# cinemere/evacuation

Measured on NVIDIA B200. Metric: pedestrian-steps/s, higher is better.
Workload: dtype f32

## Files before the change

evacuation_b200/_native.py:

```python
from __future__ import annotations

import ctypes as C
import os

from . import build as _build
from .build import LIB_PATH

EVAC_ABI_VERSION = 5
NUM_EPISODE_STATS = 9
EPISODE_STAT_KEYS = (
    "episode_intrinsic_reward", "episode_status_reward", "episode_reward", "episode_length",
    "escaped_pedestrians", "exiting_pedestrians", "following_pedestrians", "viscek_pedestrians",
    "overall_timesteps",
)

POS = {"abs": 0, "rel": 1, "grav": 2}
STAT = {"no": 0, "ohe": 1, "cat": 2}
OBS = {"Dict": 0, "Box": 1}
PREC = {"fp32": 0, "fp64": 1}
AGENT = {"table": 0, "random": 1, "rotating": 2, "wacuum": 3}
SEARCH = {"auto": 0, "brute": 1, "cells": 2}


class EvacConfig(C.Structure):
# ... 27 lines not shown
    _fields_ = [
        ("num_envs", C.c_int32), ("obs", C.c_void_p),
        ("norm_mean", C.c_void_p), ("norm_var", C.c_void_p), ("norm_count", C.c_void_p), ("obs_norm", C.c_void_p),
        ("norm_eps", C.c_float), ("norm_clip", C.c_float),
        ("embedding", C.c_void_p), ("mean", C.c_void_p), ("value", C.c_void_p), ("action", C.c_void_p),
        ("action_clipped", C.c_void_p), ("logprob", C.c_void_p), ("entropy", C.c_void_p), ("given_action", C.c_void_p),
        ("sample", C.c_int32), ("training", C.c_int32), ("seed", C.c_uint64), ("offset", C.c_uint64),
        ("offset_device", C.c_void_p), ("env_index_offset", C.c_int64),
    ]


_P = C.c_void_p
SIGNATURES = {
    "evac_abi_version": (C.c_int32, []),
    "evac_last_error": (C.c_char_p, []),
    "evac_build_id": (C.c_char_p, []),
    "evac_default_config": (C.c_int, [C.POINTER(EvacConfig)]),
    "evac_create": (C.c_int, [C.POINTER(EvacConfig), C.c_int32, C.c_int32, C.c_uint64, C.c_int64, C.POINTER(_P)]),
    "evac_destroy": (C.c_int, [_P]),
    "evac_obs_dim": (C.c_int32, [_P]),
    "evac_num_envs": (C.c_int32, [_P]),
    "evac_num_cells": (C.c_int32, [_P]),
    "evac_state_elem_size": (C.c_int32, [_P]),
    "evac_reset": (C.c_int, [_P, _P, _P, _P]),
    "evac_set_state": (C.c_int, [_P, _P, _P, _P, _P, _P, _P, _P]),
    "evac_get_state": (C.c_int, [_P, _P, _P, _P, _P, _P, _P, _P]),
    "evac_observe": (C.c_int, [_P, _P, _P]),
    "evac_step": (C.c_int, [_P, _P, _P, _P, _P, _P, _P, _P]),
    "evac_step_host": (C.c_int, [_P, _P, _P, _P, _P, _P, _P, _P]),
    "evac_rollout": (C.c_int, [_P, C.c_int32, C.c_int32, _P, _P, _P, C.c_int32, _P, _P, _P, _P, _P]),
    "evac_episode_stats": (C.c_int, [_P, _P, _P, _P, _P]),
    "evac_get_accumulators": (C.c_int, [_P, _P, _P, _P]),
    "evac_launch_count": (C.c_int64, [_P]),
    "evac_state_bytes": (C.c_int64, [_P]),
    "evac_save_state": (C.c_int, [_P, _P, _P]),
    "evac_load_state": (C.c_int, [_P, _P, _P]),
    "evac_policy_default_config": (C.c_int, [C.POINTER(EvacPolicyConfig), C.c_int32, C.c_int32]),
    "evac_policy_create": (C.c_int, [C.POINTER(EvacPolicyConfig), C.c_int32, C.POINTER(_P)]),
    "evac_policy_destroy": (C.c_int, [_P]),
    "evac_policy_num_weights": (C.c_int64, [_P]),
    "evac_policy_load_weights": (C.c_int, [_P, _P, C.c_int64]),
    "evac_policy_reserve": (C.c_int, [_P, C.c_int32]),
    "evac_policy_forward": (C.c_int, [_P, C.POINTER(EvacPolicyIO), _P]),
    "evac_policy_launch_count": (C.c_int64, [_P]),
    "evac_normalize_reward": (C.c_int, [C.c_int32, _P, _P, _P, _P, _P, _P, _P, _P, _P, C.c_float, C.c_float, C.c_float, _P]),
    "evac_probe_fma": (C.c_int, [C.c_int32, C.c_int32, C.c_int32, C.POINTER(C.c_float), C.POINTER(C.c_double)]),
    "evac_probe_pairwise": (C.c_int, [C.c_int32, C.c_int32, C.c_int32, C.c_int32, C.POINTER(C.c_float), C.POINTER(C.c_double)]),
}

_lib = None


def build_id() -> str:
    return load().evac_build_id().decode()


class EvacNativeError(RuntimeError):
    pass


def load() -> C.CDLL:
    global _lib
    if _lib is not None:
        return _lib
    want = _build.source_hash()
    if _build.library_build_id() != want and not os.environ.get("EVAC_B200_LIB"):
# ... 31 lines not shown
```

evacuation_b200/csrc/evac_abi.cu:

```cuda
#include <cuda_runtime.h>
#include <math.h>
#include <stdarg.h>
#include <stdio.h>
#include <stdlib.h>
#include <string.h>

#include <new>

#include "../../include/evac_b200.h"
#include "evac_kernels.cuh"
#include "evac_warp.cuh"

using namespace evac;

static thread_local char g_err[512] = "";

static int fail(int code, const char* fmt, ...) {
  va_list ap;
  va_start(ap, fmt);
  vsnprintf(g_err, sizeof(g_err), fmt, ap);
  va_end(ap);
  return code;
}

// ... 12 lines not shown
  EvacConfig cfg;
  int E, N, device, obs_dim, prec;
  uint64_t seed;
  long long env_offset;
  void* pos = nullptr;
  void* dir = nullptr;
  uint8_t* status = nullptr;
  float2* agent_pos = nullptr;
  float2* agent_dir = nullptr;
  int* now = nullptr;
  int* episode = nullptr;
  long long* overall = nullptr;
  double* acc = nullptr;
  float* ep_stats = nullptr;
  uint8_t* ep_finished = nullptr;
  double* totals = nullptr;
  int* agent_state = nullptr;
  unsigned char* blocks = nullptr;
  cudaStream_t stream = nullptr;
  float *h_actions = nullptr, *h_noise = nullptr, *h_obs = nullptr, *h_reward = nullptr;
  const void* pin_key[7] = {nullptr, nullptr, nullptr, nullptr, nullptr, nullptr, nullptr};
  bool pin_val[7] = {false, false, false, false, false, false, false};
  uint8_t *h_term = nullptr, *h_trunc = nullptr;
  float *d_actions = nullptr, *d_noise = nullptr, *d_obs = nullptr, *d_reward = nullptr;
  uint8_t *d_term = nullptr, *d_trunc = nullptr, *d_status = nullptr, *h_status = nullptr;
  int64_t launches = 0;
  int threads = 0, ppt = 0;
  int num_sms = 0;
  int cells_x = 0, cells_y = 0, cell_reach = 1;
  int cell_pair_walk = 1;
  int cluster = 1;
  bool warp_kernel = true;
  int warps_per_cta = 1;
};

static double sq_boundary(double t) {
  double v = t * t;
  while (v > 0 && sqrt(nextafter(v, 0.0)) >= t) v = nextafter(v, 0.0);
  while (sqrt(v) < t) v = nextafter(v, INFINITY);
  return v;
}
static float round_up_f32(double b) {
  float f = (float)b;
  if ((double)f < b) f = nextafterf(f, INFINITY);
  return f;
}
template <typename real> static real thr2_of(double t);
template <> float thr2_of<float>(double t) { return round_up_f32(sq_boundary(t)); }
template <> double thr2_of<double>(double t) { return sq_boundary(t); }

static int compute_obs_dim(const EvacConfig& c) {
  const int n = c.number_of_pedestrians;
  if (c.positions == EVAC_POS_GRAV) return 6;
  const int sc = c.statuses == EVAC_STAT_OHE ? 4 : (c.statuses == EVAC_STAT_CAT ? 1 : 0);
  if (c.obs_type == EVAC_OBS_BOX) return (n + 2) * (2 + sc);
  return 4 + 2 * n + sc * n;
}

template <typename real>
static KArgs<real> make_args(const EvacHandle* h) {
  const EvacConfig& c = h->cfg;
  KArgs<real> a;
  memset(&a, 0, sizeof(a));
  a.E = h->E; a.N = h->N; a.obs_dim = h->obs_dim;
  a.width = (real)c.width; a.height = (real)c.height; a.step_size = (real)c.step_size; a.noise_coef = (real)c.noise_coef;
  a.enslaving = (real)c.enslaving_degree; a.one_minus_enslaving = (real)(1.0 - c.enslaving_degree);
// ... 61 lines not shown
  }
  cudaLaunchConfig_t cfg = {};
  cfg.gridDim = dim3((unsigned)a.E * CL);
  cfg.blockDim = dim3(THREADS);
  cfg.dynamicSmemBytes = smem;
  cfg.stream = st;
  cudaLaunchAttribute at[1];
  at[0].id = cudaLaunchAttributeClusterDimension;
  at[0].val.clusterDim.x = CL; at[0].val.clusterDim.y = 1; at[0].val.clusterDim.z = 1;
  cfg.attrs = at;
  cfg.numAttrs = 1;
  CK(cudaLaunchKernelEx(&cfg, kern, a));
  h->launches++;
  return EVAC_OK;
}

static void pick_shape(int n, int* threads, int* ppt) {
  const char* shape = getenv("EVAC_SHAPE_64");
  if (n <= 64 && shape && strcmp(shape, "64x1") == 0) { *threads = 64; *ppt = 1; }
  else if (n <= 64) { *threads = 32; *ppt = 2; }
  else if (n <= 128) { *threads = 128; *ppt = 1; }
  else if (n <= 256) { *threads = 256; *ppt = 1; }
  else if (n <= 512) { *threads = 256; *ppt = 2; }
  else if (n <= 1024) { *threads = 512; *ppt = 2; }
  else if (n <= 2048) { *threads = 512; *ppt = 4; }
  else if (n <= 4096) {
    const char* s4 = getenv("EVAC_SHAPE_4096");
    if (s4 && strcmp(s4, "512x8") == 0) { *threads = 512; *ppt = 8; } else { *threads = 1024; *ppt = 4; }
  }
  else { *threads = 1024; *ppt = 8; }
}

template <int WPC>
static void launch_warp_t(const KArgs<float>& a, cudaStream_t st) {
  const int grid = (a.E + WPC - 1) / WPC;
  if (a.positions == POS_REL && a.statuses == STAT_OHE && a.obs_type == OBS_BOX) evac_warp_kernel<WMODE_REL_OHE_BOX, WPC><<<grid, 32 * WPC, 0, st>>>(a);
  else if (a.positions == POS_GRAV) evac_warp_kernel<WMODE_GRAV, WPC><<<grid, 32 * WPC, 0, st>>>(a);
  else evac_warp_kernel<WMODE_GENERIC, WPC><<<grid, 32 * WPC, 0, st>>>(a);
}
static int launch_warp(EvacHandle* h, const KArgs<float>& a, cudaStream_t st) {
  switch (h->warps_per_cta) {
    case 2: launch_warp_t<2>(a, st); break;
    case 4: launch_warp_t<4>(a, st); break;
    case 8: launch_warp_t<8>(a, st); break;
    default: launch_warp_t<1>(a, st); break;
  }
  CK(cudaGetLastError());
  h->launches++;
  return EVAC_OK;
}

template <typename real>
static int launch_step(EvacHandle* h, const KArgs<real>& a, cudaStream_t st) {
  if constexpr (std::is_same<real, float>::value) {
    if (h->threads == 32 && h->warp_kernel) return launch_warp(h, a, st);
    switch (h->cluster) {
      case 2: return launch_cluster_t<2>(h, a, st);
      case 4: return launch_cluster_t<4>(h, a, st);
      case 8: return launch_cluster_t<8>(h, a, st);
    }
  }
  switch (h->threads * 16 + h->ppt) {
    case 32 * 16 + 2: return launch_step_t<real, 32, 2>(h, a, st);
    case 64 * 16 + 1: return launch_step_t<real, 64, 1>(h, a, st);
    case 128 * 16 + 1: return launch_step_t<real, 128, 1>(h, a, st);
    case 256 * 16 + 1: return launch_step_t<real, 256, 1>(h, a, st);
    case 256 * 16 + 2: return launch_step_t<real, 256, 2>(h, a, st);
    case 512 * 16 + 2: return launch_step_t<real, 512, 2>(h, a, st);
    case 512 * 16 + 4: return launch_step_t<real, 512, 4>(h, a, st);
    case 512 * 16 + 8:
      if constexpr (std::is_same<real, float>::value) return launch_step_t<real, 512, 8>(h, a, st);
      break;
    case 1024 * 16 + 4: return launch_step_t<real, 1024, 4>(h, a, st);
    case 1024 * 16 + 8:
      if constexpr (std::is_same<real, float>::value) return launch_step_t<real, 1024, 8>(h, a, st);
      break;
  }
  return fail(EVAC_ERR_INVALID, "no kernel shape for N=%d", h->N);
}

// ... 57 lines not shown
  if (cfg->neighbor_search < EVAC_SEARCH_AUTO || cfg->neighbor_search > EVAC_SEARCH_CELLS) return fail(EVAC_ERR_INVALID, "invalid neighbor_search");
  if (!(cfg->to_leader > 0 && cfg->to_pedestrian > 0 && cfg->to_exit > 0 && cfg->to_escape > 0))
    return fail(EVAC_ERR_INVALID, "switch distances must be positive");
  if (cfg->max_timesteps < 1 || cfg->max_timesteps > (1 << 21)) return fail(EVAC_ERR_INVALID, "max_timesteps must be in 1 .. 2^21 (the step index is a 21-bit field of the Philox counter)");
  int ndev = 0;
  if (cudaGetDeviceCount(&ndev) != cudaSuccess || ndev == 0) {
    cudaGetLastError();
    return fail(EVAC_ERR_NO_DEVICE, "no CUDA device available; this library has no CPU fallback");
  }
  if (device < 0 || device >= ndev) return fail(EVAC_ERR_INVALID, "device %d out of range (0..%d)", device, ndev - 1);
  CK(cudaSetDevice(device));
  cudaDeviceProp prop;
  CK(cudaGetDeviceProperties(&prop, device));
  if (prop.major < 10) return fail(EVAC_ERR_NO_DEVICE, "device %d is sm_%d%d; this library is built for sm_100a (B200) only", device, prop.major, prop.minor);

  EvacHandle* h = new (std::nothrow) EvacHandle();
  if (!h) return fail(EVAC_ERR_INVALID, "out of host memory");
  h->cfg = *cfg; h->E = num_envs; h->N = cfg->number_of_pedestrians; h->device = device;
  h->obs_dim = compute_obs_dim(*cfg); h->prec = cfg->precision; h->seed = seed; h->env_offset = env_index_offset;
  h->num_sms = prop.multiProcessorCount;
  pick_shape(h->N, &h->threads, &h->ppt);
  if (h->N > 64 && h->prec == EVAC_PREC_F32 && cfg->neighbor_search != EVAC_SEARCH_BRUTE) {
    int want = h->N <= 8192 ? 1 : (h->N <= 16384 ? 4 : 8);
    const char* cl = getenv("EVAC_CLUSTER");
    if (cl) {
      const int v = atoi(cl);
      if ((v == 2 || v == 4 || v == 8) && v * 4096 >= h->N) want = v;
      if (v == 1 && h->N <= 8192) want = 1;
    }
    h->cluster = want;
    if (h->cluster > 1) { h->threads = 1024; h->ppt = 4; }
  }
  { const char* wk = getenv("EVAC_WARP_KERNEL"); h->warp_kernel = !(wk && strcmp(wk, "generic") == 0); }
  { const char* wp = getenv("EVAC_WARP_WPC"); if (wp) h->warps_per_cta = atoi(wp); }
  if (h->N > 64 && h->threads > 32 && h->prec == EVAC_PREC_F32 && cfg->neighbor_search != EVAC_SEARCH_BRUTE) {
    const char* rs = getenv("EVAC_CELL_REACH");
    int reach = (rs && atoi(rs) == 1) ? 1 : 2;
    double edge = cfg->to_pedestrian * (1.0 + 1e-4) / reach;
    if (2.0 * cfg->width / edge > 64.0 || 2.0 * cfg->height / edge > 64.0) { reach = 1; edge = cfg->to_pedestrian * (1.0 + 1e-4); }
    int gx = (int)fmin(64.0, floor(2.0 * cfg->width / edge)), gy = (int)fmin(64.0, floor(2.0 * cfg->height / edge));
    {
      const size_t budget = (size_t)prop.sharedMemPerBlockOptin - 4096 , slots = (size_t)h->threads * h->ppt;
      while (gx * gy > 16 && Tile<float>::bytes((int)slots) + CellSmem::bytes((int)slots, gx * gy) > budget) { gx = (gx * 7 + 7) / 8; gy = (gy * 7 + 7) / 8; }
      while (h->cluster > 1 && gx * gy > 2048) { gx = (gx * 7 + 7) / 8; gy = (gy * 7 + 7) / 8; }
    }
    if (gx >= 1 && gy >= 1 && (cfg->neighbor_search == EVAC_SEARCH_CELLS || gx * gy >= 16 || h->cluster > 1)) { h->cells_x = gx; h->cells_y = gy; h->cell_reach = reach; }
    h->cell_pair_walk = 2 * h->N >= gx * gy;
    { const char* pw = getenv("EVAC_CELL_PAIR_WALK"); if (pw) h->cell_pair_walk = atoi(pw) != 0; }
    { const char* dy = getenv("EVAC_CELL_DYNAMIC"); if (h->cell_pair_walk && dy && atoi(dy) == 1) h->cell_pair_walk |= 2; }
    { const char* gr = getenv("EVAC_CELL_GROUP"); if (h->cell_pair_walk && h->cluster == 1 && gr && atoi(gr) == 1) h->cell_pair_walk |= 4; }
  } else if (h->threads == 32 && h->prec == EVAC_PREC_F32 && cfg->neighbor_search == EVAC_SEARCH_CELLS) {
    const int gx = (int)fmin(32.0, floor(2.0 * cfg->width / (cfg->to_pedestrian * (1.0 + 1e-4))));
    if (gx >= 1) { h->cells_x = gx; h->cells_y = 1; }
  }
  const size_t en = (size_t)h->E * h->N, es = h->prec == EVAC_PREC_F64 ? 16 : 8;
#define ALLOC(ptr, bytes)                                                      \
  do {                                                                         \
    cudaError_t _e = cudaMalloc((void**)&(ptr), (bytes));                      \
    if (_e != cudaSuccess) { evac_destroy(h); return fail(EVAC_ERR_CUDA, "cudaMalloc(%zu) failed: %s", (size_t)(bytes), cudaGetErrorString(_e)); } \
    cudaMemset((ptr), 0, (bytes));                                             \
  } while (0)
  if (h->threads == 32 && h->warp_kernel && h->prec == EVAC_PREC_F32) {
    ALLOC(h->blocks, (size_t)h->E * BLK_BYTES);
  } else {
    ALLOC(h->pos, en * es); ALLOC(h->dir, en * es); ALLOC(h->status, en);
    ALLOC(h->agent_pos, (size_t)h->E * sizeof(float2)); ALLOC(h->agent_dir, (size_t)h->E * sizeof(float2));
    ALLOC(h->now, (size_t)h->E * sizeof(int)); ALLOC(h->episode, (size_t)h->E * sizeof(int));
    ALLOC(h->overall, (size_t)h->E * sizeof(long long)); ALLOC(h->acc, (size_t)h->E * 3 * sizeof(double));
    ALLOC(h->agent_state, (size_t)h->E * sizeof(int));
  }
  ALLOC(h->ep_stats, (size_t)h->E * EVAC_NUM_EPISODE_STATS * sizeof(float)); ALLOC(h->ep_finished, (size_t)h->E);
  ALLOC(h->totals, (1 + EVAC_NUM_EPISODE_STATS) * sizeof(double));
#undef ALLOC
  CK(cudaStreamCreateWithFlags(&h->stream, cudaStreamNonBlocking));
  CK(cudaDeviceSynchronize());
  *out = h;
  return EVAC_OK;
}

int evac_destroy(EvacHandle* h) {
  if (!h) return EVAC_OK;
  cudaSetDevice(h->device);
  cudaDeviceSynchronize();
  void* dptrs[] = {h->pos, h->dir, h->status, h->agent_pos, h->agent_dir, h->now, h->episode, h->overall, h->acc,
                   h->ep_stats, h->ep_finished, h->totals, h->agent_state, h->blocks, h->d_actions, h->d_noise, h->d_obs };
  for (void* p : dptrs) if (p) cudaFree(p);
  void* hptrs[] = {h->h_actions, h->h_noise, h->h_obs };
  for (void* p : hptrs) if (p) cudaFreeHost(p);
  if (h->stream) cudaStreamDestroy(h->stream);
  delete h;
  return EVAC_OK;
}

int32_t evac_obs_dim(const EvacHandle* h) { return h ? h->obs_dim : -1; }
int32_t evac_num_cells(const EvacHandle* h) { return h ? h->cells_x * h->cells_y : -1; }
int32_t evac_num_envs(const EvacHandle* h) { return h ? h->E : -1; }
int32_t evac_state_elem_size(const EvacHandle* h) { return h ? (h->prec == EVAC_PREC_F64 ? 8 : 4) : -1; }
int64_t evac_launch_count(const EvacHandle* h) { return h ? h->launches : -1; }

int evac_reset(EvacHandle* h, const uint8_t* reset_mask, float* obs, void* stream) {
  if (!h) return fail(EVAC_ERR_INVALID, "NULL handle");
  if (int r = set_device(h)) return r;
  cudaStream_t st = (cudaStream_t)stream;
  const int flags = AUX_RESET | (obs ? AUX_OBS : 0);
  return h->prec == EVAC_PREC_F64 ? launch_aux<double>(h, flags, reset_mask, obs, st) : launch_aux<float>(h, flags, reset_mask, obs, st);
}

int evac_observe(EvacHandle* h, float* obs, void* stream) {
  if (!h || !obs) return fail(EVAC_ERR_INVALID, "NULL argument");
  if (int r = set_device(h)) return r;
  cudaStream_t st = (cudaStream_t)stream;
  return h->prec == EVAC_PREC_F64 ? launch_aux<double>(h, AUX_OBS, nullptr, obs, st) : launch_aux<float>(h, AUX_OBS, nullptr, obs, st);
}

int evac_set_state(EvacHandle* h, const void* positions, const void* directions, const uint8_t* statuses,
                   const float* agent_position, const float* agent_direction, const int32_t* now, void* stream) {
  if (!h) return fail(EVAC_ERR_INVALID, "NULL handle");
  if (int r = set_device(h)) return r;
  cudaStream_t st = (cudaStream_t)stream;
  const size_t en = (size_t)h->E * h->N, es = h->prec == EVAC_PREC_F64 ? 16 : 8;
  if (h->blocks) {
    StateIO io = {(float2*)positions, (float2*)directions, (uint8_t*)statuses, (float2*)agent_position, (float2*)agent_direction, (int*)now, nullptr, nullptr};
    evac_block_io_kernel<true><<<h->E, 64, 0, st>>>(h->blocks, h->E, h->N, io);
    CK(cudaGetLastError());
    h->launches++;
    if (!statuses && (positions || agent_position)) return launch_aux<float>(h, AUX_STATUS, nullptr, nullptr, st);
    return EVAC_OK;
  }
  if (positions) CK(cudaMemcpyAsync(h->pos, positions, en * es, cudaMemcpyDeviceToDevice, st));
  if (directions) CK(cudaMemcpyAsync(h->dir, directions, en * es, cudaMemcpyDeviceToDevice, st));
  if (agent_position) CK(cudaMemcpyAsync(h->agent_pos, agent_position, (size_t)h->E * 8, cudaMemcpyDeviceToDevice, st));
// ... 2 lines not shown
  if (agent_position) CK(cudaMemsetAsync(h->agent_state, 0, (size_t)h->E * sizeof(int), st));
  if (statuses) {
    CK(cudaMemcpyAsync(h->status, statuses, en, cudaMemcpyDeviceToDevice, st));
  } else if (positions || agent_position) {
    return h->prec == EVAC_PREC_F64 ? launch_aux<double>(h, AUX_STATUS, nullptr, nullptr, st) : launch_aux<float>(h, AUX_STATUS, nullptr, nullptr, st);
  }
  return EVAC_OK;
}

int evac_get_state(EvacHandle* h, void* positions, void* directions, uint8_t* statuses, float* agent_position,
                   float* agent_direction, int32_t* now, void* stream) {
  if (!h) return fail(EVAC_ERR_INVALID, "NULL handle");
  if (int r = set_device(h)) return r;
  cudaStream_t st = (cudaStream_t)stream;
  const size_t en = (size_t)h->E * h->N, es = h->prec == EVAC_PREC_F64 ? 16 : 8;
  if (h->blocks) {
    StateIO io = {(float2*)positions, (float2*)directions, statuses, (float2*)agent_position, (float2*)agent_direction, now, nullptr, nullptr};
    evac_block_io_kernel<false><<<h->E, 64, 0, st>>>(h->blocks, h->E, h->N, io);
    CK(cudaGetLastError());
    h->launches++;
    return EVAC_OK;
  }
  if (positions) CK(cudaMemcpyAsync(positions, h->pos, en * es, cudaMemcpyDeviceToDevice, st));
  if (directions) CK(cudaMemcpyAsync(directions, h->dir, en * es, cudaMemcpyDeviceToDevice, st));
  if (statuses) CK(cudaMemcpyAsync(statuses, h->status, en, cudaMemcpyDeviceToDevice, st));
  if (agent_position) CK(cudaMemcpyAsync(agent_position, h->agent_pos, (size_t)h->E * 8, cudaMemcpyDeviceToDevice, st));
  if (agent_direction) CK(cudaMemcpyAsync(agent_direction, h->agent_dir, (size_t)h->E * 8, cudaMemcpyDeviceToDevice, st));
  if (now) CK(cudaMemcpyAsync(now, h->now, (size_t)h->E * 4, cudaMemcpyDeviceToDevice, st));
  return EVAC_OK;
}

static int rollout_impl(EvacHandle* h, int32_t num_steps, int32_t agent_kind, const float* actions, const float* noise, float* obs,
                        int32_t obs_every_step, float* reward_sum, uint8_t* terminated, uint8_t* truncated, uint16_t* status_counts,
                        uint8_t* status_out, void* stream) {
  if (!h) return fail(EVAC_ERR_INVALID, "NULL handle");
  if (num_steps < 1) return fail(EVAC_ERR_INVALID, "num_steps must be >= 1");
  if (agent_kind < EVAC_AGENT_TABLE || agent_kind > EVAC_AGENT_WACUUM) return fail(EVAC_ERR_INVALID, "invalid agent_kind");
  if (agent_kind == EVAC_AGENT_TABLE && !actions) return fail(EVAC_ERR_INVALID, "actions is NULL");
  if (int r = set_device(h)) return r;
  cudaStream_t st = (cudaStream_t)stream;
  if (h->prec == EVAC_PREC_F64) {
    KArgs<double> a = make_args<double>(h);
    a.actions = (const float2*)actions; a.noise = noise; a.obs = obs; a.obs_every_step = obs_every_step;
    a.reward = reward_sum; a.terminated = terminated; a.truncated = truncated; a.num_steps = num_steps; a.agent_kind = agent_kind;
    a.status_counts = status_counts; a.status_out = status_out;
    return launch_step<double>(h, a, st);
  }
  KArgs<float> a = make_args<float>(h);
  a.actions = (const float2*)actions; a.noise = noise; a.obs = obs; a.obs_every_step = obs_every_step;
  a.reward = reward_sum; a.terminated = terminated; a.truncated = truncated; a.num_steps = num_steps; a.agent_kind = agent_kind;
  a.status_counts = status_counts; a.status_out = status_out;
  return launch_step<float>(h, a, st);
}

int evac_rollout(EvacHandle* h, int32_t num_steps, int32_t agent_kind, const float* actions, const float* noise, float* obs,
                 int32_t obs_every_step, float* reward_sum, uint8_t* terminated, uint8_t* truncated, uint16_t* status_counts,
                 void* stream) {
  return rollout_impl(h, num_steps, agent_kind, actions, noise, obs, obs_every_step, reward_sum, terminated, truncated, status_counts, nullptr, stream);
}

int evac_step(EvacHandle* h, const float* actions, const float* noise, float* obs, float* reward, uint8_t* terminated,
              uint8_t* truncated, void* stream) {
  if (!actions) return fail(EVAC_ERR_INVALID, "actions is NULL");
  return evac_rollout(h, 1, EVAC_AGENT_TABLE, actions, noise, obs, 0, reward, terminated, truncated, nullptr, stream);
}

static bool is_pinned(const void* p) {
  if (!p) return false;
  cudaPointerAttributes attr;
  if (cudaPointerGetAttributes(&attr, p) != cudaSuccess) { cudaGetLastError(); return false; }
  return attr.type == cudaMemoryTypeHost;
}

int evac_step_host(EvacHandle* h, const float* actions, const float* noise, float* obs, float* reward, uint8_t* terminated,
                   uint8_t* truncated, uint8_t* statuses) {
  if (!h || !actions) return fail(EVAC_ERR_INVALID, "NULL argument");
  if (int r = set_device(h)) return r;
  const size_t E = h->E, N = h->N, D = h->obs_dim;
  if (!h->h_actions) {
    CK(cudaMallocHost((void**)&h->h_actions, E * 8)); CK(cudaMalloc((void**)&h->d_actions, E * 8));
    const size_t out_bytes = E * D * 4 + E * 4 + 2 * E + E * N;
    unsigned char *hb = nullptr, *db = nullptr;
    CK(cudaMallocHost((void**)&hb, out_bytes)); CK(cudaMalloc((void**)&db, out_bytes));
    h->h_obs = (float*)hb; h->h_reward = (float*)(hb + E * D * 4); h->h_term = hb + E * D * 4 + E * 4; h->h_trunc = h->h_term + E; h->h_status = h->h_trunc + E;
    h->d_obs = (float*)db; h->d_reward = (float*)(db + E * D * 4); h->d_term = db + E * D * 4 + E * 4; h->d_trunc = h->d_term + E; h->d_status = h->d_trunc + E;
  }
  if (noise && !h->h_noise) { CK(cudaMallocHost((void**)&h->h_noise, E * N * 4)); CK(cudaMalloc((void**)&h->d_noise, E * N * 4)); }
  cudaStream_t st = h->stream;
  const void* ptrs[7] = {actions, noise, obs, reward, terminated, truncated, statuses};
  for (int i = 0; i < 7; ++i)
    if (ptrs[i] != h->pin_key[i]) { h->pin_key[i] = ptrs[i]; h->pin_val[i] = is_pinned(ptrs[i]); }
  const bool pa = h->pin_val[0], pn = h->pin_val[1], po = h->pin_val[2], pr = h->pin_val[3], pt = h->pin_val[4], pu = h->pin_val[5], ps = h->pin_val[6];
  {
    static const bool zc_on = [] { const char* z = getenv("EVAC_HOST_ZEROCOPY"); return !(z && z[0] == '0'); }();
    static const size_t zc_max = [] { const char* z = getenv("EVAC_HOST_ZEROCOPY_BYTES"); return z ? (size_t)atoll(z) : (size_t)1 << 20; }();
    const size_t bytes = E * (D * 4 + 14 + N * 5);
    if (zc_on && bytes <= zc_max && pa && (!noise || pn) && (!obs || po) && (!reward || pr) && (!terminated || pt) && (!truncated || pu) &&
        (!statuses || ps)) {
      if (int r = rollout_impl(h, 1, EVAC_AGENT_TABLE, actions, noise, obs, 0, reward ? reward : h->d_reward, terminated ? terminated : h->d_term,
                               truncated ? truncated : h->d_trunc, nullptr, statuses, st)) return r;
      CK(cudaStreamSynchronize(st));
      return EVAC_OK;
    }
  }
  static const bool act_zc = [] { const char* z = getenv("EVAC_HOST_ACTIONS_ZEROCOPY"); return !(z && z[0] == '0'); }();
  const float* act_dev = h->d_actions;
  if (pa && act_zc) act_dev = actions;
  else {
    if (!pa) memcpy(h->h_actions, actions, E * 8);
    CK(cudaMemcpyAsync(h->d_actions, pa ? actions : h->h_actions, E * 8, cudaMemcpyHostToDevice, st));
  }
  if (noise) {
    if (!pn) memcpy(h->h_noise, noise, E * N * 4);
    CK(cudaMemcpyAsync(h->d_noise, pn ? noise : h->h_noise, E * N * 4, cudaMemcpyHostToDevice, st));
  }
  if (int r = rollout_impl(h, 1, EVAC_AGENT_TABLE, act_dev, noise ? h->d_noise : nullptr, obs ? h->d_obs : nullptr, 0, h->d_reward, h->d_term,
                           h->d_trunc, nullptr, statuses ? h->d_status : nullptr, st)) return r;
  const size_t head_bytes = E * D * 4 + E * 4 + 2 * E;
  const bool packed = reward == obs + E * D && terminated == (uint8_t*)(reward + E) && truncated == terminated + E &&
                      (!statuses || statuses == truncated + E);
  const bool packed_pinned = po && pr && pt && pu && (!statuses || ps) && obs && packed;
  const bool all_pageable = !po && !pr && !pt && !pu && !ps && obs && reward && terminated && truncated;
  if (packed_pinned || all_pageable) {
    CK(cudaMemcpyAsync(packed_pinned ? (void*)obs : (void*)h->h_obs, h->d_obs, head_bytes + (statuses ? E * N : 0), cudaMemcpyDeviceToHost, st));
  } else {
    if (obs) CK(cudaMemcpyAsync(po ? obs : h->h_obs, h->d_obs, E * D * 4, cudaMemcpyDeviceToHost, st));
    if (reward) CK(cudaMemcpyAsync(pr ? reward : h->h_reward, h->d_reward, E * 4, cudaMemcpyDeviceToHost, st));
    if (terminated) CK(cudaMemcpyAsync(pt ? terminated : h->h_term, h->d_term, E, cudaMemcpyDeviceToHost, st));
    if (truncated) CK(cudaMemcpyAsync(pu ? truncated : h->h_trunc, h->d_trunc, E, cudaMemcpyDeviceToHost, st));
    if (statuses) CK(cudaMemcpyAsync(ps ? statuses : h->h_status, h->d_status, E * N, cudaMemcpyDeviceToHost, st));
  }
  CK(cudaStreamSynchronize(st));
  if (obs && !po) memcpy(obs, h->h_obs, E * D * 4);
  if (reward && !pr) memcpy(reward, h->h_reward, E * 4);
  if (terminated && !pt) memcpy(terminated, h->h_term, E);
  if (truncated && !pu) memcpy(truncated, h->h_trunc, E);
  if (statuses && !ps) memcpy(statuses, h->h_status, E * N);
  return EVAC_OK;
}

int evac_get_accumulators(EvacHandle* h, double* acc, int64_t* overall_timesteps, void* stream) {
  if (!h) return fail(EVAC_ERR_INVALID, "NULL handle");
  if (int r = set_device(h)) return r;
  cudaStream_t st = (cudaStream_t)stream;
  if (h->blocks) {
    StateIO io = {nullptr, nullptr, nullptr, nullptr, nullptr, nullptr, acc, (long long*)overall_timesteps};
    evac_block_io_kernel<false><<<h->E, 64, 0, st>>>(h->blocks, h->E, h->N, io);
    CK(cudaGetLastError());
    h->launches++;
    return EVAC_OK;
// ... 302 lines not shown
```

evacuation_b200/csrc/evac_kernels.cuh:

```cuda
#pragma once
#include <cooperative_groups.h>
#include <cuda_runtime.h>
#include <math.h>
#include <stdint.h>

#include <type_traits>

#include "philox.cuh"

namespace evac {

constexpr int ST_NONE = 0, ST_VISCEK = 1, ST_FOLLOWER = 2, ST_EXITING = 3, ST_ESCAPED = 4;
constexpr int POS_ABS = 0, POS_REL = 1, POS_GRAV = 2;
constexpr int STAT_NO = 0, STAT_OHE = 1, STAT_CAT = 2;
constexpr int OBS_DICT = 0, OBS_BOX = 1;
constexpr int AGENT_TABLE = 0, AGENT_RANDOM = 1, AGENT_ROTATING = 2, AGENT_WACUUM = 3;
constexpr int NUM_EPISODE_STATS = 9;
constexpr float PARK = 1.0e18f;

template <typename real> struct vec2;
template <> struct vec2<float> { using type = float2; };
template <> struct vec2<double> { using type = double2; };

template <typename real>
struct KArgs {
  int E, N, obs_dim;
  real width, height, step_size, noise_coef, enslaving, one_minus_enslaving;
  float width_f, height_f, step_size_f, eps_f, enslaving_f;
  real thr2_ped, thr2_leader, thr2_exit, thr2_escape;
  int cells_x, cells_y, cell_reach;
  int cell_pair_walk;
  float cell_inv_x, cell_inv_y;
  int exit_reward, follow_reward, term_wall;
  real init_reward, intrinsic_coef;
  int max_timesteps;
  real inv_200n, inv_n;
  int positions, statuses, obs_type;
  real alpha, eps;
  int alpha_plus2_int;
  int auto_reset;
  typename vec2<real>::type* pos;
  typename vec2<real>::type* dir;
  uint8_t* status;
  float2* agent_pos;
  float2* agent_dir;
  int* now;
  int* episode;
  long long* overall;
  double* acc;
  float* ep_stats;
  uint8_t* ep_finished;
  double* totals;
  int* agent_state;
  unsigned char* blocks;
  float wac_top, wac_right, wac_left, wac_bottom;
  const float2* actions;
  const float* noise;
  float* obs;
  int obs_every_step;
  float* reward;
  uint8_t* terminated;
  uint8_t* truncated;
  uint16_t* status_counts;
  uint8_t* status_out;
  int num_steps, agent_kind;
  uint64_t seed;
  long long env_offset;
};

struct __align__(16) EnvRec {
  float2 agent_pos, agent_dir;
  int now, episode, agent_state, pad;
  long long overall;
  double acc[3];
};
static_assert(sizeof(EnvRec) == 64, "EnvRec is one 64-byte record");
constexpr int BLK_STATUS = 64, BLK_PED = 128, BLK_SLOTS = 64, BLK_BYTES = BLK_PED + 16 * BLK_SLOTS;
__host__ __device__ __forceinline__ int blk_status_off(int i) { return BLK_STATUS + 2 * (i & 31) + (i >> 5); }

template <typename real>
__device__ __forceinline__ void state_load_ped(const KArgs<real>& a, int e, int i, real& px, real& py, real& dx, real& dy, int& st) {
  if constexpr (std::is_same<real, float>::value) {
    if (a.blocks != nullptr) {
      const unsigned char* b = a.blocks + (size_t)e * BLK_BYTES;
      const float4 v = reinterpret_cast<const float4*>(b + BLK_PED)[i];
      px = v.x; py = v.y; dx = v.z; dy = v.w;
      st = b[blk_status_off(i)];
      return;
    }
// ... 1152 lines not shown
```

evacuation_b200/csrc/evac_warp.cuh:

```cuda
#pragma once
#include "evac_kernels.cuh"

namespace evac {

enum { WMODE_GENERIC = 0, WMODE_REL_OHE_BOX = 1, WMODE_GRAV = 2 };

__device__ __forceinline__ float2 splat(float v) { return make_float2(v, v); }

__device__ __forceinline__ void windowed_pass(const Tile<float>& t, int j0, int j1, float x, float y, float thr2, float& sx, float& sy) {
  const float2 nx = splat(-x), ny = splat(-y);
  float2 ax = make_float2(0.f, 0.f), ay = make_float2(0.f, 0.f);
  if (j0 < j1) {
    float4 p = t.P2[j0], u = t.U2[j0];
#pragma unroll 2
    for (int j = j0; j < j1; ++j) {
      const float4 pn = t.P2[j + 1], un = t.U2[j + 1];
      const float2 dx = __fadd2_rn(make_float2(p.x, p.y), nx);
      const float2 dy = __fadd2_rn(make_float2(p.z, p.w), ny);
      float2 d2 = __fmul2_rn(dx, dx);
      d2 = __ffma2_rn(dy, dy, d2);
      const float2 w = make_float2(d2.x < thr2 ? 1.f : 0.f, d2.y < thr2 ? 1.f : 0.f);
      ax = __ffma2_rn(w, make_float2(u.x, u.y), ax);
      ay = __ffma2_rn(w, make_float2(u.z, u.w), ay);
      p = pn;
      u = un;
    }
  }
  sx = ax.x + ax.y;
  sy = ay.x + ay.y;
}

struct WPed {
  float2 p, d;
  int st;
};

#ifndef EVAC_WARP_MINB
#define EVAC_WARP_MINB 28
#endif
#ifndef EVAC_PAIR_UNROLL
#define EVAC_PAIR_UNROLL 4
#endif
template <int MODE, int WPC>
__global__ void __launch_bounds__(32 * WPC, EVAC_WARP_MINB / WPC) evac_warp_kernel(const __grid_constant__ KArgs<float> a) {
#if defined(EVAC_OBS_STAGED) || defined(EVAC_OBS_BULK)
  __shared__ __align__(128) float4 tile_all[WPC][99];
#else
  __shared__ __align__(16) float4 tile_all[WPC][66];
#endif
  __shared__ uint2 strip_mask_all[WPC][32];
  __shared__ int strip_start_all[WPC][33];
  const int wic = threadIdx.x >> 5;
  const int lane = threadIdx.x & 31, e = blockIdx.x * WPC + wic, N = a.N;
  if (e >= a.E) return;
#ifdef EVAC_PROBE_EMPTY
  if (a.N >= 0) return;
#endif
  const Tile<float> tile(reinterpret_cast<unsigned char*>(tile_all[wic]), 64);
  uint2* strip_mask = strip_mask_all[wic];
  int* strip_start = strip_start_all[wic];
  const int S = a.cells_x;
  const uint32_t lt_mask = (1u << lane) - 1u;
  const bool valid[2] = {lane < N, lane + 32 < N};
  const uint32_t env_g = (uint32_t)(a.env_offset + e);
  const float2 exit_p = make_float2(0.f, -1.f);

  unsigned char* const blk = a.blocks + (size_t)e * BLK_BYTES;
  float4* const ped_l = reinterpret_cast<float4*>(blk + BLK_PED) + lane;
  unsigned short* const st_l = reinterpret_cast<unsigned short*>(blk + BLK_STATUS) + lane;
  const float4 pd0 = ped_l[0], pd1 = ped_l[32];
  const unsigned st2 = *st_l;
  const float4 rec0 = *reinterpret_cast<const float4*>(blk);
  const int4 rec1 = *reinterpret_cast<const int4*>(blk + 16);
  const longlong2 rec2 = *reinterpret_cast<const longlong2*>(blk + 32);
  long long overall = rec2.x;
  double acc_r = __longlong_as_double(rec2.y), acc_i = 0, acc_s = 0;
  if (lane == 0) {
    const double2 r3 = *reinterpret_cast<const double2*>(blk + 48);
    acc_i = r3.x; acc_s = r3.y;
  }
  WPed q[2];
  q[0].p = make_float2(pd0.x, pd0.y); q[0].d = make_float2(pd0.z, pd0.w); q[0].st = (int)(st2 & 0xffu);
  q[1].p = make_float2(pd1.x, pd1.y); q[1].d = make_float2(pd1.z, pd1.w); q[1].st = (int)(st2 >> 8);
  float2 ap = make_float2(rec0.x, rec0.y), ad = make_float2(rec0.z, rec0.w);
  int now = rec1.x, episode = rec1.y, wac_state = rec1.z;
  float reward_sum = 0.f;
  int any_term = 0, any_trunc = 0;
// ... 351 lines not shown
```

evacuation_b200/env.py:

```python
from __future__ import annotations

import ctypes as C
import logging
import os
from typing import Optional

import numpy as np
import torch

from . import _native as nat
from .config import EnvConfig
from .spaces import Box, Dict
from .statuses import Status, SwitchDistances

log = logging.getLogger(__name__)

_TORCH_STATE_DTYPE = {"fp32": torch.float32, "fp64": torch.float64}


def _ptr(t: Optional[torch.Tensor]):
    return None if t is None else C.c_void_p(t.data_ptr())


class _Pedestrians:
# ... 210 lines not shown
        self._obs_view = self._structure(self._obs)
        self._host = None
        return h

    def close(self):
        if self._h is not None:
            torch.cuda.synchronize(self.device)
            nat.load().evac_destroy(self._h)
            self._h = None

    def __del__(self):
        try:
            self.close()
        except Exception:
            pass

    @property
    def obs_dim(self) -> int:
        self._handle()
        return self._obs_dim

    @property
    def flat_observation(self) -> torch.Tensor:
        self._handle()
        return self._obs

    @property
    def num_cells(self) -> int:
        return int(nat.load().evac_num_cells(self._handle()))

    @property
    def launch_count(self) -> int:
        return int(nat.load().evac_launch_count(self._handle()))

    def get_state(self) -> dict:
        h, lib = self._handle(), nat.load()
        E, N, dev = self.num_envs, self.cfg.number_of_pedestrians, self.device
        dt = _TORCH_STATE_DTYPE[self.precision]
        st = dict(positions=torch.empty((E, N, 2), dtype=dt, device=dev),
                  directions=torch.empty((E, N, 2), dtype=dt, device=dev),
                  statuses=torch.empty((E, N), dtype=torch.uint8, device=dev),
                  agent_position=torch.empty((E, 2), dtype=torch.float32, device=dev),
                  agent_direction=torch.empty((E, 2), dtype=torch.float32, device=dev),
                  now=torch.empty(E, dtype=torch.int32, device=dev))
        nat.check(lib.evac_get_state(h, _ptr(st["positions"]), _ptr(st["directions"]), _ptr(st["statuses"]),
                                     _ptr(st["agent_position"]), _ptr(st["agent_direction"]), _ptr(st["now"]),
                                     self._stream()))
        return st

    def set_state(self, positions=None, directions=None, statuses=None, agent_position=None,
                  agent_direction=None, now=None):
        h, lib = self._handle(), nat.load()
        E, N, dev = self.num_envs, self.cfg.number_of_pedestrians, self.device
        dt = _TORCH_STATE_DTYPE[self.precision]

        def prep(x, shape, dtype):
            if x is None:
                return None
            t = torch.as_tensor(np.asarray(x) if not torch.is_tensor(x) else x)
            return t.to(device=dev, dtype=dtype).reshape(shape).contiguous()

        p, d = prep(positions, (E, N, 2), dt), prep(directions, (E, N, 2), dt)
        s = prep(statuses, (E, N), torch.uint8)
        ap, ad = prep(agent_position, (E, 2), torch.float32), prep(agent_direction, (E, 2), torch.float32)
        nw = prep(now, (E,), torch.int32)
        nat.check(lib.evac_set_state(h, _ptr(p), _ptr(d), _ptr(s), _ptr(ap), _ptr(ad), _ptr(nw), self._stream()))
# ... 263 lines not shown
```

include/evac_b200.h:

```cpp
#ifndef EVAC_B200_H_
#define EVAC_B200_H_

#include <stdint.h>

#ifdef __cplusplus
extern "C" {
#endif

#define EVAC_ABI_VERSION 5

enum {
  EVAC_OK = 0,
  EVAC_ERR_INVALID = -1,
  EVAC_ERR_CUDA = -2,
  EVAC_ERR_UNSUPPORTED = -3,
  EVAC_ERR_NO_DEVICE = -4
};

enum { EVAC_STATUS_VISCEK = 1, EVAC_STATUS_FOLLOWER = 2, EVAC_STATUS_EXITING = 3, EVAC_STATUS_ESCAPED = 4 };
enum { EVAC_POS_ABS = 0, EVAC_POS_REL = 1, EVAC_POS_GRAV = 2 };
enum { EVAC_STAT_NO = 0, EVAC_STAT_OHE = 1, EVAC_STAT_CAT = 2 };
enum { EVAC_OBS_DICT = 0, EVAC_OBS_BOX = 1 };
enum { EVAC_PREC_F32 = 0, EVAC_PREC_F64 = 1 };
enum { EVAC_AGENT_TABLE = 0, EVAC_AGENT_RANDOM = 1, EVAC_AGENT_ROTATING = 2, EVAC_AGENT_WACUUM = 3 };
// ... 39 lines not shown
int32_t evac_num_envs(const EvacHandle* h);
int32_t evac_num_cells(const EvacHandle* h);
int32_t evac_state_elem_size(const EvacHandle* h);

int evac_reset(EvacHandle* h, const uint8_t* reset_mask, float* obs, void* stream);

int evac_set_state(EvacHandle* h, const void* positions, const void* directions, const uint8_t* statuses,
                   const float* agent_position, const float* agent_direction, const int32_t* now, void* stream);
int evac_get_state(EvacHandle* h, void* positions, void* directions, uint8_t* statuses,
                   float* agent_position, float* agent_direction, int32_t* now, void* stream);

int evac_observe(EvacHandle* h, float* obs, void* stream);

int evac_step(EvacHandle* h, const float* actions, const float* noise, float* obs, float* reward,
              uint8_t* terminated, uint8_t* truncated, void* stream);

int evac_step_host(EvacHandle* h, const float* actions, const float* noise, float* obs, float* reward,
                   uint8_t* terminated, uint8_t* truncated, uint8_t* statuses);

int64_t evac_state_bytes(EvacHandle* h);
int evac_save_state(EvacHandle* h, void* image, void* stream);
int evac_load_state(EvacHandle* h, const void* image, void* stream);

int evac_rollout(EvacHandle* h, int32_t num_steps, int32_t agent_kind, const float* actions, const float* noise,
                 float* obs, int32_t obs_every_step, float* reward_sum, uint8_t* terminated, uint8_t* truncated,
                 uint16_t* status_counts, void* stream);

int evac_episode_stats(EvacHandle* h, float* stats, uint8_t* finished, double* totals, void* stream);

int evac_get_accumulators(EvacHandle* h, double* acc, int64_t* overall_timesteps, void* stream);

int64_t evac_launch_count(const EvacHandle* h);

const char* evac_last_error(void);
int32_t evac_abi_version(void);

typedef struct EvacPolicyConfig {
  int32_t abi_version;
  int32_t seq_len;
  int32_t d_model;
  int32_t num_heads;
  int32_t dim_feedforward;
  int32_t num_blocks;
  int32_t use_resid;
  float dropout;
  float layer_norm_eps;
  int32_t num_hidden;
  int32_t action_dim;
} EvacPolicyConfig;

typedef struct EvacPolicy EvacPolicy;

int evac_policy_default_config(EvacPolicyConfig* cfg, int32_t number_of_pedestrians, int32_t d_model);
int evac_policy_create(const EvacPolicyConfig* cfg, int32_t device, EvacPolicy** out);
int evac_policy_destroy(EvacPolicy* p);
int64_t evac_policy_num_weights(const EvacPolicy* p);
int evac_policy_load_weights(EvacPolicy* p, const float* weights, int64_t count);
int evac_policy_reserve(EvacPolicy* p, int32_t max_envs);

typedef struct EvacPolicyIO {
  int32_t num_envs;
  const float* obs;
  float* norm_mean;
  float* norm_var;
  const double* norm_count;
  float* obs_norm;
// ... 31 lines not shown
```

Measured before the change: 24.86 billion.

## Launch warp step kernel with programmatic dependent launch and L2 prefetch

```diff
diff --git a/evacuation_b200/_native.py b/evacuation_b200/_native.py
--- a/evacuation_b200/_native.py
+++ b/evacuation_b200/_native.py
@@ -83,6 +83,7 @@
     "evac_episode_stats": (C.c_int, [_P, _P, _P, _P, _P]),
     "evac_get_accumulators": (C.c_int, [_P, _P, _P, _P]),
     "evac_launch_count": (C.c_int64, [_P]),
+    "evac_pdl": (C.c_int32, [_P]),
     "evac_state_bytes": (C.c_int64, [_P]),
     "evac_save_state": (C.c_int, [_P, _P, _P]),
     "evac_load_state": (C.c_int, [_P, _P, _P]),
diff --git a/evacuation_b200/csrc/evac_abi.cu b/evacuation_b200/csrc/evac_abi.cu
--- a/evacuation_b200/csrc/evac_abi.cu
+++ b/evacuation_b200/csrc/evac_abi.cu
@@ -68,6 +68,9 @@
   int cluster = 1;
   bool warp_kernel = true;
   int warps_per_cta = 1;
+  const void* warp_fn = nullptr;
+  bool pdl = false;
+  int warp_smem = 0;
 };
 
 static double sq_boundary(double t) {
@@ -195,20 +198,33 @@
 }
 
 template <int WPC>
-static void launch_warp_t(const KArgs<float>& a, cudaStream_t st) {
-  const int grid = (a.E + WPC - 1) / WPC;
-  if (a.positions == POS_REL && a.statuses == STAT_OHE && a.obs_type == OBS_BOX) evac_warp_kernel<WMODE_REL_OHE_BOX, WPC><<<grid, 32 * WPC, 0, st>>>(a);
-  else if (a.positions == POS_GRAV) evac_warp_kernel<WMODE_GRAV, WPC><<<grid, 32 * WPC, 0, st>>>(a);
-  else evac_warp_kernel<WMODE_GENERIC, WPC><<<grid, 32 * WPC, 0, st>>>(a);
+static const void* warp_kernel_t(const EvacConfig& c) {
+  if (c.positions == EVAC_POS_REL && c.statuses == EVAC_STAT_OHE && c.obs_type == EVAC_OBS_BOX) return (const void*)evac_warp_kernel<WMODE_REL_OHE_BOX, WPC>;
+  if (c.positions == EVAC_POS_GRAV) return (const void*)evac_warp_kernel<WMODE_GRAV, WPC>;
+  return (const void*)evac_warp_kernel<WMODE_GENERIC, WPC>;
+}
+static const void* warp_kernel(const EvacConfig& c, int wpc) {
+  switch (wpc) {
+    case 2: return warp_kernel_t<2>(c);
+    case 4: return warp_kernel_t<4>(c);
+    case 8: return warp_kernel_t<8>(c);
+    default: return warp_kernel_t<1>(c);
+  }
 }
 static int launch_warp(EvacHandle* h, const KArgs<float>& a, cudaStream_t st) {
-  switch (h->warps_per_cta) {
-    case 2: launch_warp_t<2>(a, st); break;
-    case 4: launch_warp_t<4>(a, st); break;
-    case 8: launch_warp_t<8>(a, st); break;
-    default: launch_warp_t<1>(a, st); break;
-  }
-  CK(cudaGetLastError());
+  const int wpc = h->warps_per_cta;
+  cudaLaunchConfig_t cfg = {};
+  cfg.gridDim = dim3((unsigned)((a.E + wpc - 1) / wpc));
+  cfg.blockDim = dim3(32 * wpc);
+  cfg.dynamicSmemBytes = h->warp_smem;
+  cfg.stream = st;
+  cudaLaunchAttribute at[1];
+  at[0].id = cudaLaunchAttributeProgrammaticStreamSerialization;
+  at[0].val.programmaticStreamSerializationAllowed = 1;
+  cfg.attrs = at;
+  cfg.numAttrs = h->pdl ? 1 : 0;
+  void* args[] = {const_cast<KArgs<float>*>(&a)};
+  CK(cudaLaunchKernelExC(&cfg, h->warp_fn, args));
   h->launches++;
   return EVAC_OK;
 }
@@ -332,7 +348,7 @@
     if (h->cluster > 1) { h->threads = 1024; h->ppt = 4; }
   }
   { const char* wk = getenv("EVAC_WARP_KERNEL"); h->warp_kernel = !(wk && strcmp(wk, "generic") == 0); }
-  { const char* wp = getenv("EVAC_WARP_WPC"); if (wp) h->warps_per_cta = atoi(wp); }
+  { const char* wp = getenv("EVAC_WARP_WPC"); const int v = wp ? atoi(wp) : 1; h->warps_per_cta = (v == 2 || v == 4 || v == 8) ? v : 1; }
   if (h->N > 64 && h->threads > 32 && h->prec == EVAC_PREC_F32 && cfg->neighbor_search != EVAC_SEARCH_BRUTE) {
     const char* rs = getenv("EVAC_CELL_REACH");
     int reach = (rs && atoi(rs) == 1) ? 1 : 2;
@@ -372,6 +388,30 @@
   ALLOC(h->ep_stats, (size_t)h->E * EVAC_NUM_EPISODE_STATS * sizeof(float)); ALLOC(h->ep_finished, (size_t)h->E);
   ALLOC(h->totals, (1 + EVAC_NUM_EPISODE_STATS) * sizeof(double));
 #undef ALLOC
+  if (h->blocks) {
+    h->warp_fn = warp_kernel(*cfg, h->warps_per_cta);
+    { const char* pd = getenv("EVAC_PDL"); h->pdl = !(pd && pd[0] == '0'); }
+    const char* pin = getenv("EVAC_PDL_PIN");
+    if (h->pdl && !(pin && pin[0] == '0')) {
+      const int threads = 32 * h->warps_per_cta, grid = (h->E + h->warps_per_cta - 1) / h->warps_per_cta;
+      const int per_sm = (grid + h->num_sms - 1) / h->num_sms;
+      int natural = 0;
+      CK(cudaOccupancyMaxActiveBlocksPerMultiprocessor(&natural, h->warp_fn, threads, 0));
+      if (per_sm < natural) {
+        cudaFuncAttributes fa;
+        CK(cudaFuncGetAttributes(&fa, h->warp_fn));
+        int lo = 0, hi = (int)(prop.sharedMemPerBlockOptin - fa.sharedSizeBytes);
+        CK(cudaFuncSetAttribute(h->warp_fn, cudaFuncAttributeMaxDynamicSharedMemorySize, hi));
+        while (lo < hi) {
+          const int mid = (lo + hi) / 2;
+          int occ = 0;
+          CK(cudaOccupancyMaxActiveBlocksPerMultiprocessor(&occ, h->warp_fn, threads, mid));
+          if (occ <= per_sm) hi = mid; else lo = mid + 1;
+        }
+        h->warp_smem = lo;
+      }
+    }
+  }
   CK(cudaStreamCreateWithFlags(&h->stream, cudaStreamNonBlocking));
   CK(cudaDeviceSynchronize());
   *out = h;
@@ -397,6 +437,7 @@
 int32_t evac_num_envs(const EvacHandle* h) { return h ? h->E : -1; }
 int32_t evac_state_elem_size(const EvacHandle* h) { return h ? (h->prec == EVAC_PREC_F64 ? 8 : 4) : -1; }
 int64_t evac_launch_count(const EvacHandle* h) { return h ? h->launches : -1; }
+int32_t evac_pdl(const EvacHandle* h) { return h ? (int32_t)h->pdl : -1; }
 
 int evac_reset(EvacHandle* h, const uint8_t* reset_mask, float* obs, void* stream) {
   if (!h) return fail(EVAC_ERR_INVALID, "NULL handle");
@@ -465,7 +506,7 @@
 
 static int rollout_impl(EvacHandle* h, int32_t num_steps, int32_t agent_kind, const float* actions, const float* noise, float* obs,
                         int32_t obs_every_step, float* reward_sum, uint8_t* terminated, uint8_t* truncated, uint16_t* status_counts,
-                        uint8_t* status_out, void* stream) {
+                        uint8_t* status_out, bool actions_on_device, void* stream) {
   if (!h) return fail(EVAC_ERR_INVALID, "NULL handle");
   if (num_steps < 1) return fail(EVAC_ERR_INVALID, "num_steps must be >= 1");
   if (agent_kind < EVAC_AGENT_TABLE || agent_kind > EVAC_AGENT_WACUUM) return fail(EVAC_ERR_INVALID, "invalid agent_kind");
@@ -480,7 +521,7 @@
     return launch_step<double>(h, a, st);
   }
   KArgs<float> a = make_args<float>(h);
-  a.actions = (const float2*)actions; a.noise = noise; a.obs = obs; a.obs_every_step = obs_every_step;
+  a.actions = (const float2*)actions; a.actions_on_device = actions_on_device; a.noise = noise; a.obs = obs; a.obs_every_step = obs_every_step;
   a.reward = reward_sum; a.terminated = terminated; a.truncated = truncated; a.num_steps = num_steps; a.agent_kind = agent_kind;
   a.status_counts = status_counts; a.status_out = status_out;
   return launch_step<float>(h, a, st);
@@ -489,7 +530,7 @@
 int evac_rollout(EvacHandle* h, int32_t num_steps, int32_t agent_kind, const float* actions, const float* noise, float* obs,
                  int32_t obs_every_step, float* reward_sum, uint8_t* terminated, uint8_t* truncated, uint16_t* status_counts,
                  void* stream) {
-  return rollout_impl(h, num_steps, agent_kind, actions, noise, obs, obs_every_step, reward_sum, terminated, truncated, status_counts, nullptr, stream);
+  return rollout_impl(h, num_steps, agent_kind, actions, noise, obs, obs_every_step, reward_sum, terminated, truncated, status_counts, nullptr, true, stream);
 }
 
 int evac_step(EvacHandle* h, const float* actions, const float* noise, float* obs, float* reward, uint8_t* terminated,
@@ -531,7 +572,7 @@
     if (zc_on && bytes <= zc_max && pa && (!noise || pn) && (!obs || po) && (!reward || pr) && (!terminated || pt) && (!truncated || pu) &&
         (!statuses || ps)) {
       if (int r = rollout_impl(h, 1, EVAC_AGENT_TABLE, actions, noise, obs, 0, reward ? reward : h->d_reward, terminated ? terminated : h->d_term,
-                               truncated ? truncated : h->d_trunc, nullptr, statuses, st)) return r;
+                               truncated ? truncated : h->d_trunc, nullptr, statuses, false, st)) return r;
       CK(cudaStreamSynchronize(st));
       return EVAC_OK;
     }
@@ -548,7 +589,7 @@
     CK(cudaMemcpyAsync(h->d_noise, pn ? noise : h->h_noise, E * N * 4, cudaMemcpyHostToDevice, st));
   }
   if (int r = rollout_impl(h, 1, EVAC_AGENT_TABLE, act_dev, noise ? h->d_noise : nullptr, obs ? h->d_obs : nullptr, 0, h->d_reward, h->d_term,
-                           h->d_trunc, nullptr, statuses ? h->d_status : nullptr, st)) return r;
+                           h->d_trunc, nullptr, statuses ? h->d_status : nullptr, act_dev == h->d_actions, st)) return r;
   const size_t head_bytes = E * D * 4 + E * 4 + 2 * E;
   const bool packed = reward == obs + E * D && terminated == (uint8_t*)(reward + E) && truncated == terminated + E &&
                       (!statuses || statuses == truncated + E);
diff --git a/evacuation_b200/csrc/evac_kernels.cuh b/evacuation_b200/csrc/evac_kernels.cuh
--- a/evacuation_b200/csrc/evac_kernels.cuh
+++ b/evacuation_b200/csrc/evac_kernels.cuh
@@ -55,6 +55,7 @@
   unsigned char* blocks;
   float wac_top, wac_right, wac_left, wac_bottom;
   const float2* actions;
+  int actions_on_device;
   const float* noise;
   float* obs;
   int obs_every_step;
diff --git a/evacuation_b200/csrc/evac_warp.cuh b/evacuation_b200/csrc/evac_warp.cuh
--- a/evacuation_b200/csrc/evac_warp.cuh
+++ b/evacuation_b200/csrc/evac_warp.cuh
@@ -53,6 +53,14 @@
   const int wic = threadIdx.x >> 5;
   const int lane = threadIdx.x & 31, e = blockIdx.x * WPC + wic, N = a.N;
   if (e >= a.E) return;
+  {
+    const void* pf = nullptr;
+    if (lane < BLK_BYTES / 128) pf = a.blocks + (size_t)e * BLK_BYTES + 128 * lane;
+    else if (lane == BLK_BYTES / 128 && a.agent_kind == AGENT_TABLE && a.actions_on_device) pf = a.actions + e;
+    if (pf != nullptr) asm volatile("prefetch.global.L2 [%0];" ::"l"(pf) : "memory");
+  }
+  asm volatile("griddepcontrol.launch_dependents;" ::: "memory");
+  asm volatile("griddepcontrol.wait;" ::: "memory");
 #ifdef EVAC_PROBE_EMPTY
   if (a.N >= 0) return;
 #endif
diff --git a/evacuation_b200/env.py b/evacuation_b200/env.py
--- a/evacuation_b200/env.py
+++ b/evacuation_b200/env.py
@@ -266,6 +266,10 @@
     @property
     def launch_count(self) -> int:
         return int(nat.load().evac_launch_count(self._handle()))
+
+    @property
+    def pdl(self) -> bool:
+        return bool(nat.load().evac_pdl(self._handle()) == 1)
 
     def get_state(self) -> dict:
         h, lib = self._handle(), nat.load()
diff --git a/include/evac_b200.h b/include/evac_b200.h
--- a/include/evac_b200.h
+++ b/include/evac_b200.h
@@ -95,6 +95,8 @@
 
 int64_t evac_launch_count(const EvacHandle* h);
 
+int32_t evac_pdl(const EvacHandle* h);
+
 const char* evac_last_error(void);
 int32_t evac_abi_version(void);
 
```

New measurement: 27.42 billion (median of 6 runs). 1.1x the previous value.
